# MayeulCassier/Matrix-Factorization-With-Comparison-Data

Hardware: AMD Instinct MI355X
Metric: triplet-updates/sec (higher is better)
Workload: dtype f32

## Files before the change

matrix-factorization-with-comparison-data_amd/csrc/resident.hip:

```cpp
#include <cstring>
#include <mutex>
#include <utility>
#include <vector>

#include "resident_kernel.h"

#define MFCD_DECL(d)                                                                                                  \
    extern "C" int mfcd_resident_launch_d##d(const mfcd_detail::ResidentArgs *, int, int, void *) __attribute__((weak)); \
    extern "C" int mfcd_resident_occupancy_d##d(int, int, int, int) __attribute__((weak));
MFCD_DECL(2) MFCD_DECL(4) MFCD_DECL(8) MFCD_DECL(16) MFCD_DECL(32) MFCD_DECL(64) MFCD_DECL(128) MFCD_DECL(256)
#undef MFCD_DECL

namespace mfcd_detail {

int g_resident_math = 1;
Tuning g_tune;

typedef int (*ResidentLauncher)(const ResidentArgs *, int, int, void *);
typedef int (*ResidentOccupancy)(int, int, int, int);

static ResidentLauncher launcher_for(int d)
{
    switch (d) {
        case 2: return mfcd_resident_launch_d2;
// ... 141 lines not shown
    for (int r = 0; r < 3; ++r) {
        bool first = true;
#pragma unroll
        for (int r2 = 0; r2 < r; ++r2) first = first && w[r2] != w[r];
        need[r] = first;
        unsigned own = 0u, rows = 0u;
#pragma unroll
        for (int r2 = r; r2 < 3; ++r2)
            if (w[r2] == w[r]) {
                own |= 1u << r2;
                rows |= lr[r2] << (10 * r2);
            }
        e[r] = make_uint4(((unsigned)k << 9) | (tl << 3) | own, rows, __float_as_uint(s.z), 0u);
        list[r] = (size_t)w[r] * (size_t)nch_cap + (size_t)c;
    }
    unsigned slot[3] = {0u, 0u, 0u}, slot_back[3] = {0u, 0u, 0u};
#pragma unroll
    for (int r = 0; r < 3; ++r) {
        if (need[r]) slot[r] = atomicAdd(ev_cnt + list[r], 1u);
        if (need[r] && copy_back) slot_back[r] = atomicAdd(ev_cnt + list[r] - 1, 1u);
    }
#pragma unroll
    for (int r = 0; r < 3; ++r) {
        if (need[r] && slot[r] < (unsigned)kEventCap - 1u) ev_ent[list[r] * kEventCap + slot[r]] = e[r];
        if (need[r] && copy_back && slot_back[r] < (unsigned)kEventCap - 1u)
            ev_ent[(list[r] - 1) * kEventCap + slot_back[r]] = e[r];
    }
}

int launch_train_prologue(const StageCopy &sc, const SampleTranslation *tr, hipStream_t st)
{
    static const SampleTranslation none{nullptr, 0, 1, 0, 0, 0, 0, 0, 0, nullptr, nullptr, nullptr};
    const SampleTranslation &t = tr ? *tr : none;
    const int units = (int)((sc.bytes + 15) / 16);
    const int64_t items = t.xs ? (t.N > units ? t.N : units) : units;
    constexpr int kPT = 64;
    const dim3 grid((unsigned)((items + kPT - 1) / kPT));
    if (units <= kInlineStageUnits) {
        InlineStage inl;
        std::memcpy(inl.v, sc.host, (size_t)units * 16);
        hipLaunchKernelGGL(train_prologue_kernel<true>, grid, dim3(kPT), 0, st, inl, (const uint4 *)nullptr,
                           (uint4 *)sc.dev, units, t.samples, t.N, t.B, t.n, t.m, t.rows_per_wave, t.tshift, t.look,
                           t.nch_cap, t.xs, t.ev_cnt, (uint4 *)t.ev_ent);
    } else {
        static const InlineStage no_inline{};
        hipLaunchKernelGGL(train_prologue_kernel<false>, grid, dim3(kPT), 0, st, no_inline, (const uint4 *)sc.devview,
                           (uint4 *)sc.dev, units, t.samples, t.N, t.B, t.n, t.m, t.rows_per_wave, t.tshift, t.look,
                           t.nch_cap, t.xs, t.ev_cnt, (uint4 *)t.ev_ent);
    }
    MFCD_HIP_TRY(hipGetLastError());
    return 0;
}

int launch_resident_steps(const ResidentPlan &pl, const void *cold_dev, const mfcd_sample *xs, int64_t N, int B, int n,
                          int m, int d, const StepScalars *sc_dev, const AdamStatic &ac, unsigned long long *mailbox,
                          unsigned tag_base, void *loss_terms, unsigned long long *dbg, int K, hipStream_t st)
{
    ResidentArgs a;
    a.dbg = dbg;
    a.cold = (const ResidentCold *)cold_dev;
    a.samples = xs; a.sc = sc_dev; a.mailbox = mailbox; a.loss_terms = loss_terms;
    a.N = N; a.B = B; a.n = n; a.m = m; a.K = K; a.NW = pl.NW; a.ac = ac;
    a.lookahead = pl.lookahead;
    a.tag_base = tag_base;
    a.fast_math = pl.fast_math;
    a.bf16 = pl.bf16;
    ResidentLauncher fn = launcher_for(d);
    if (!fn) return MFCD_EINVAL;
    return fn(&a, pl.Q, pl.blocks, (void *)st);
}

}
```

matrix-factorization-with-comparison-data_amd/csrc/resident_kernel.h:

```cpp
#pragma once
#include "common.h"
#include "train_common.h"

namespace mfcd_detail {

typedef unsigned long long u64;

#define MFCD_LAMBDA_INLINE __attribute__((always_inline))

#ifdef MFCD_RES_STATS
#define RS_NOW() ((u64)__builtin_amdgcn_s_memtime())
#define RS_ADD(slot, val) rs_acc[slot] += (u64)(val)
#else
#define RS_NOW() ((u64)0)
#define RS_ADD(slot, val) ((void)0)
#endif

typedef const __attribute__((address_space(4))) float *ScalarTablePtr;
__device__ __forceinline__ StepScalars load_step_scalars(const StepScalars *table, int k)
{
    const ScalarTablePtr f = (ScalarTablePtr)(table + k);
    StepScalars s;
    s.neg_step_size = f[0];
    s.bc2_sqrt = f[1];
    s.inv_bc2_sqrt = f[2];
    s.pad = 0.0f;
    return s;
}


__device__ __forceinline__ u64 pack_granule(unsigned tag, float v)
{
    return ((u64)tag << 32) | (u64)__float_as_uint(v);
}

__device__ __forceinline__ u64 load_granule(const u64 *p)
{
    return __hip_atomic_load(p, __ATOMIC_RELAXED, __HIP_MEMORY_SCOPE_AGENT);
}

__device__ __forceinline__ void store_granule(u64 *p, unsigned tag, float v)
{
    __hip_atomic_store(p, pack_granule(tag, v), __ATOMIC_RELAXED, __HIP_MEMORY_SCOPE_AGENT);
}

struct RowMap {
    int n, m, c;
    __host__ __device__ int vrow_u(int u) const { return u < c ? 2 * u : 2 * c + (u - c); }
    __host__ __device__ int vrow_v(int i) const { return i < c ? 2 * i + 1 : 2 * c + (i - c); }
    __host__ __device__ int users_below(int x) const
    {
        if (x <= 2 * c) return (x + 1) >> 1;
        return n > c ? c + (x - 2 * c) : c;
    }
    __host__ __device__ int items_below(int x) const
    {
        if (x <= 2 * c) return x >> 1;
        return m > c ? c + (x - 2 * c) : c;
    }
    __host__ __device__ bool is_item(int vr) const { return vr < 2 * c ? (vr & 1) != 0 : m > n; }
    __host__ __device__ int table_row(int vr) const { return vr < 2 * c ? vr >> 1 : c + (vr - 2 * c); }
};
__host__ __device__ inline RowMap make_row_map(int n, int m)
{
    RowMap r;
    r.n = n; r.m = m; r.c = n < m ? n : m;
    return r;
}

constexpr int kEventCap = 64;
constexpr unsigned kEventNone = 0xFFFFFFF8u;
constexpr int kEventMaxLocalRows = 1024;

struct ResidentArgs {
    const ResidentCold *cold;
    const mfcd_sample *samples;
    const StepScalars *sc;
    u64 *mailbox;
    void *loss_terms;
    u64 *dbg;
    unsigned tag_base;
    int64_t N;
    int B, n, m, K, NW;
    int lookahead;
    int fast_math;
    int bf16;
    AdamStatic ac;
};

__device__ __forceinline__ mfcd_sample load_record(const mfcd_sample *__restrict__ samples, int64_t pos0, int Bk,
                                                   int base, int lane)
{
    mfcd_sample s;
    s.u = s.i = s.j = -0x40000000;
    s.z = 0.0f;
    if (base + lane < Bk) s = samples[pos0 + base + lane];
    return s;
}

struct Masks {
    u64 mu, mi, mj;
};

template <int D, int Q, int LOOK, bool FAST, bool BF16 = false>
__global__ __launch_bounds__(256) __attribute__((amdgpu_waves_per_eu(Q >= 16 ? 2 : 1)))
void resident_train_kernel(ResidentArgs a)
{
    constexpr int S = D >= 64 ? D / 64 : 1;
    constexpr int RPR = D < 64 ? 64 / D : 1;
    constexpr int EW = 64 * Q;
    static_assert(EW % D == 0, "a wave's slice must hold whole rows");
    static_assert(EW / D <= kEventMaxLocalRows, "local row indices are 10-bit fields of an event entry");
    constexpr bool GRL = Q >= 16;
    extern __shared__ __attribute__((aligned(16))) float lds_dyn[];
    const int lane = threadIdx.x & 63;
    const int gw = blockIdx.x * (blockDim.x >> 6) + (threadIdx.x >> 6);
    if (gw >= a.NW) return;

    const int64_t T = (int64_t)(a.n + a.m) * D;
    const int64_t ebase = (int64_t)gw * EW;
    const int Rlo = (int)(ebase / D);
    const int64_t eend = (ebase + EW < T) ? ebase + EW : T;
    const int Rhi = (int)(eend / D);
    const int lcol = lane & (D - 1);
    auto elem_is_item = [&](int64_t e) MFCD_LAMBDA_INLINE { return make_row_map(a.n, a.m).is_item((int)(e / D)); };
    auto elem_offset = [&](int64_t e) MFCD_LAMBDA_INLINE { return (int64_t)make_row_map(a.n, a.m).table_row((int)(e / D)) * D + (e % D); };

#ifdef MFCD_RES_STATS
    u64 rs_acc[8] = {0, 0, 0, 0, 0, 0, 0, 0};
    const u64 rs_t0 = RS_NOW();
    [[maybe_unused]] const u64 rs_abs_t0 = __builtin_amdgcn_s_memrealtime();
    [[maybe_unused]] u64 rs_abs_l0 = 0, rs_abs_l1 = 0;
    [[maybe_unused]] u64 rs_hit[8] = {0, 0, 0, 0, 0, 0, 0, 0};
    [[maybe_unused]] u64 rs_mark = 0;
#endif
    float p[Q], m1[Q], m2[Q], gr[GRL ? 1 : Q];
    float *const lgr = lds_dyn + (threadIdx.x >> 6) * (GRL ? EW : 0);
    auto post = [](float x) MFCD_LAMBDA_INLINE {
        if constexpr (BF16) return (float)(mfcd_bf16)x;
        else return x;
    };
    {
        const ResidentCold c = *a.cold;
#pragma unroll
        for (int q = 0; q < Q; ++q) {
            const int64_t e = ebase + q * 64 + lane;
            p[q] = m1[q] = m2[q] = 0.0f;
            if constexpr (GRL) lgr[q * 64 + lane] = 0.0f;
            if (e < T) {
                const int64_t o = elem_offset(e);
                if (!elem_is_item(e)) { p[q] = BF16 ? (float)((const mfcd_bf16 *)c.U)[o] : c.U[o]; m1[q] = c.mU[o]; m2[q] = c.vU[o]; }
                else { p[q] = BF16 ? (float)((const mfcd_bf16 *)c.V)[o] : c.V[o]; m1[q] = c.mV[o]; m2[q] = c.vV[o]; }
            }
        }
    }

    auto batch_size = [&](int step) MFCD_LAMBDA_INLINE {
        const int64_t pos0 = (int64_t)step * a.B;
        return (int)((a.N - pos0) < a.B ? (a.N - pos0) : a.B);
    };
    auto scan = [&](const mfcd_sample &s, int Bk, int base) MFCD_LAMBDA_INLINE {
        const bool valid = base + lane < Bk;
        const int ru = s.u, ri = s.i, rj = s.j;
        Masks M;
        M.mu = __ballot(valid && ru >= Rlo && ru < Rhi);
        M.mi = __ballot(valid && ri >= Rlo && ri < Rhi);
        M.mj = __ballot(valid && rj >= Rlo && rj < Rhi);
        return M;
    };
    auto reg_of = [&](int lr) MFCD_LAMBDA_INLINE { return D >= 64 ? lr * S : lr / RPR; };

    auto give_up = [&](int step, int64_t pos, int what) MFCD_LAMBDA_INLINE {
        int *const status = a.cold->status;
        if (lane == 0) {
            if (__hip_atomic_exchange(status, 1, __ATOMIC_RELAXED, __HIP_MEMORY_SCOPE_AGENT) == 0 && a.dbg) {
                a.dbg[0] = (u64)gw; a.dbg[1] = (u64)step; a.dbg[2] = (u64)pos; a.dbg[3] = (u64)what;
            }
        }
    };
    auto poll_failed = [&](unsigned &spins, unsigned &limit) MFCD_LAMBDA_INLINE -> bool {
        if (spins == 0) limit = (unsigned)a.cold->spin_limit;
        ++spins;
        if (spins > limit || (spins & 255u) == 0) {
            if (spins > limit ||
                __hip_atomic_load(a.cold->status, __ATOMIC_RELAXED, __HIP_MEMORY_SCOPE_AGENT) != 0)
                return true;
        }
        return false;
    };

    auto store_row = [&](int lr, int64_t slot, unsigned tag) MFCD_LAMBDA_INLINE {
        u64 *dst = a.mailbox + slot * D;
        const int q0 = reg_of(lr);
#pragma unroll
        for (int q = 0; q < Q; ++q) {
            if (q >= q0 && q < q0 + S) {
                if constexpr (D >= 64) {
                    store_granule(dst + (q - q0) * 64 + lane, tag, p[q]);
                } else {
                    if (lane / D == lr % RPR) store_granule(dst + lcol, tag, p[q]);
                }
            }
        }
    };

    auto process_hit = [&](bool own0, bool own1, bool own2, int lr0, int lr1, int lr2, float zz, int64_t pos,
                           unsigned tag, float inv_batch, int step) MFCD_LAMBDA_INLINE -> bool {
        const bool own[3] = {own0, own1, own2};
        const int lrs[3] = {lr0, lr1, lr2};
        const u64 *slot = a.mailbox + pos * 3 * D;

        float row[3][S];
#pragma unroll
        for (int r = 0; r < 3; ++r) {
#pragma unroll
            for (int s2 = 0; s2 < S; ++s2) row[r][s2] = 0.0f;
            if (!own[r]) continue;
            const int q0 = reg_of(lrs[r]);
            if constexpr (D >= 64) {
#pragma unroll
                for (int q = 0; q < Q; ++q)
                    if (q >= q0 && q < q0 + S) row[r][(q * 64 % D) / 64] = p[q];
            } else {
                float sel = 0.0f;
#pragma unroll
                for (int q = 0; q < Q; ++q) sel = (q == q0) ? p[q] : sel;
                const float v = __shfl(sel, (lrs[r] % RPR) * D + lcol, MFCD_WAVE);
                row[r][0] = lane < D ? v : 0.0f;
            }
        }
        unsigned spins = 0, limit = 0;
        [[maybe_unused]] u64 rs_w0 = 0;
        RS_ADD(4, 1ull);
#ifdef MFCD_RES_STAMPS
        { const u64 t = RS_NOW(); rs_hit[0] += t - rs_mark; rs_mark = t; }
#endif
#if defined(MFCD_RES_STAGGER) && MFCD_RES_STAGGER > 0
        {
            u64 ga[3][S], gb[3][S];
            auto issue = [&](u64 (&g)[3][S]) MFCD_LAMBDA_INLINE {
#pragma unroll
                for (int r = 0; r < 3; ++r) {
                    if (own[r]) continue;
#pragma unroll
                    for (int s2 = 0; s2 < S; ++s2) {
                        const int c = lane + 64 * s2;
                        if (c < D) g[r][s2] = load_granule(slot + (int64_t)r * D + c);
                    }
                }
            };
            auto check = [&](const u64 (&g)[3][S]) MFCD_LAMBDA_INLINE -> bool {
                bool ok = true;
#pragma unroll
                for (int r = 0; r < 3; ++r) {
                    if (own[r]) continue;
#pragma unroll
                    for (int s2 = 0; s2 < S; ++s2) {
                        const int c = lane + 64 * s2;
                        if (c < D) {
                            ok = ok && ((unsigned)(g[r][s2] >> 32) == tag);
                            row[r][s2] = __uint_as_float((unsigned)g[r][s2]);
                        }
                    }
                }
                return __all(ok);
            };
            issue(ga);
            if (!check(ga)) {
#ifdef MFCD_RES_STATS
                rs_w0 = RS_NOW();
#endif
                issue(ga);
                __builtin_amdgcn_s_sleep(MFCD_RES_STAGGER);
                issue(gb);
                while (true) {
                    RS_ADD(5, 1);
                    if (poll_failed(spins, limit)) {
                        give_up(step, pos, (own0 ? 1 : 0) | (own1 ? 2 : 0) | (own2 ? 4 : 0));
                        return false;
                    }
                    if (check(ga)) break;
                    issue(ga);
                    if (check(gb)) break;
                    issue(gb);
                }
            }
        }
#else
        while (true) {
            bool ok = true;
#pragma unroll
            for (int r = 0; r < 3; ++r) {
                if (own[r]) continue;
#pragma unroll
                for (int s2 = 0; s2 < S; ++s2) {
                    const int c = lane + 64 * s2;
                    if (c < D) {
                        const u64 gq = load_granule(slot + (int64_t)r * D + c);
                        ok = ok && ((unsigned)(gq >> 32) == tag);
                        row[r][s2] = __uint_as_float((unsigned)gq);
                    }
                }
            }
            if (__all(ok)) break;
#ifdef MFCD_RES_STATS
            if (spins == 0) rs_w0 = RS_NOW();
            RS_ADD(5, 1);
#endif
            if (poll_failed(spins, limit)) {
                give_up(step, pos, (own0 ? 1 : 0) | (own1 ? 2 : 0) | (own2 ? 4 : 0));
                return false;
            }
        }
#endif
#ifdef MFCD_RES_STATS
        if (spins) RS_ADD(2, RS_NOW() - rs_w0);
        else RS_ADD(4, 1ull << 40);
#endif
#ifdef MFCD_RES_STAMPS
        { const u64 t = RS_NOW(); rs_hit[1] += t - rs_mark; if (!spins) { rs_hit[6] += t - rs_mark; rs_hit[7] += 1; } rs_mark = t; }
#endif

        float acc = 0.0f;
#pragma unroll
        for (int s2 = 0; s2 < S; ++s2) acc += row[0][s2] * (row[1][s2] - row[2][s2]);
        float pr, g;
        if constexpr (FAST) {
            const float x = wave_sum64(acc);
            const float e = __builtin_amdgcn_exp2f(x * -1.44269504088896340736f);
            const float dn = 1.0f + e;
            pr = div_newton(1.0f, dn, __builtin_amdgcn_rcpf(dn));
            pr = (e == __builtin_inff()) ? 0.0f : pr;
            const float den = fmaxf((1.0f - pr) * pr, 1e-12f);
            const float num = inv_batch * (pr - zz);
            g = div_newton(num, den, __builtin_amdgcn_rcpf(den)) * (1.0f - pr) * pr;
        } else {
            pr = sigmoid_f32(wave_sum64(acc));
            g = bce_sigmoid_backward_f32(pr, zz, inv_batch);
        }
        if (own[0] && lane == 0) {
            if constexpr (LOOK > 0) store_granule((u64 *)a.loss_terms + pos, tag, pr);
            else ((float *)a.loss_terms)[pos] = pr;
        }

        float du[S], dv[S];
#pragma unroll
        for (int s2 = 0; s2 < S; ++s2) {
            du[s2] = g * (row[1][s2] - row[2][s2]);
            dv[s2] = g * row[0][s2];
        }
        if constexpr (D < 64) {
            du[0] = __shfl(du[0], lcol, MFCD_WAVE);
            dv[0] = __shfl(dv[0], lcol, MFCD_WAVE);
        }
        if constexpr (GRL) {
#pragma unroll
            for (int r = 0; r < 3; ++r) {
                if (!own[r]) continue;
                const int q0 = reg_of(lrs[r]);
                if constexpr (D >= 64) {
#pragma unroll
                    for (int s2 = 0; s2 < S; ++s2)
                        lgr[(q0 + s2) * 64 + lane] += r == 0 ? du[s2] : (r == 1 ? dv[s2] : -dv[s2]);
                } else {
                    if (lane / D == lrs[r] % RPR) lgr[q0 * 64 + lane] += r == 0 ? du[0] : (r == 1 ? dv[0] : -dv[0]);
                }
            }
// ... 29 lines not shown
                    adam_update_t<FAST>(p[q], m1[q], m2[q], 0.0f, a.ac, sc);
                    p[q] = post(p[q]);
                }
            }
        } else {
            adam_update_q<FAST, Q, false>(p, m1, m2, gr, a.ac, sc);
            if constexpr (BF16) {
#pragma unroll
                for (int q = 0; q < Q; ++q) p[q] = post(p[q]);
            }
        }
    };

    auto generic_loop = [&]() MFCD_LAMBDA_INLINE -> bool {
        auto publish = [&](int step) MFCD_LAMBDA_INLINE {
            const int64_t pos0 = (int64_t)step * a.B;
            const int Bk = batch_size(step);
            for (int base = 0; base < Bk; base += MFCD_WAVE) {
                const mfcd_sample s = load_record(a.samples, pos0, Bk, base, lane);
                const Masks M = scan(s, Bk, base);
                u64 mask = M.mu | M.mi | M.mj;
                while (mask) {
                    const int tl = __ffsll((long long)mask) - 1;
                    mask &= mask - 1;
                    const int64_t slot0 = (pos0 + base + tl) * 3;
                    if ((M.mu >> tl) & 1ull) store_row(__shfl(s.u, tl, MFCD_WAVE) - Rlo, slot0 + 0, a.tag_base + (unsigned)step + 1u);
                    if ((M.mi >> tl) & 1ull) store_row(__shfl(s.i, tl, MFCD_WAVE) - Rlo, slot0 + 1, a.tag_base + (unsigned)step + 1u);
                    if ((M.mj >> tl) & 1ull) store_row(__shfl(s.j, tl, MFCD_WAVE) - Rlo, slot0 + 2, a.tag_base + (unsigned)step + 1u);
                }
            }
        };
        publish(0);
        for (int k = 0; k < a.K; ++k) {
            const int64_t pos0 = (int64_t)k * a.B;
            const int Bk = batch_size(k);
            const float inv_batch = 1.0f / (float)Bk;
            const StepScalars sc = load_step_scalars(a.sc, k);
            if constexpr (!GRL) {
#pragma unroll
                for (int q = 0; q < Q; ++q) gr[q] = 0.0f;
            }
            bool any_hit = false;
            for (int base = 0; base < Bk; base += MFCD_WAVE) {
                const mfcd_sample s = load_record(a.samples, pos0, Bk, base, lane);
                const Masks M = scan(s, Bk, base);
                u64 mask = M.mu | M.mi | M.mj;
                any_hit = any_hit || mask != 0ull;
                while (mask) {
                    const int tl = __ffsll((long long)mask) - 1;
                    mask &= mask - 1;
                    const int hu = __shfl(s.u, tl, MFCD_WAVE) - Rlo, hi = __shfl(s.i, tl, MFCD_WAVE) - Rlo,
                              hj = __shfl(s.j, tl, MFCD_WAVE) - Rlo;
                    const float hz = __shfl(s.z, tl, MFCD_WAVE);
                    const bool ok = process_hit((bool)((M.mu >> tl) & 1ull), (bool)((M.mi >> tl) & 1ull),
                                                (bool)((M.mj >> tl) & 1ull), hu, hi, hj, hz, pos0 + base + tl,
                                                a.tag_base + (unsigned)k + 1u, inv_batch, k);
                    if (__builtin_amdgcn_readfirstlane((int)!ok)) return false;
                }
            }
            step_update(any_hit, sc);
            if (k + 1 < a.K) publish(k + 1);
        }
        return true;
    };

    bool alive = true;

    if constexpr (LOOK > 0) {
        const int W = __builtin_amdgcn_readfirstlane(a.lookahead);
        const int N32 = (int)a.N;
        const int gws = __builtin_amdgcn_readfirstlane(gw);
        const int tshift = (int)a.cold->tshift;
        const int NCH = ((a.K - 1) >> tshift) + 1;

        bool fits = true;
        {
            const unsigned *cnt = a.cold->ev_cnt + (size_t)gws * (size_t)a.cold->nch_cap;
            for (int c = lane; c < NCH; c += MFCD_WAVE) fits = fits && cnt[c] < (unsigned)kEventCap;
            fits = __all(fits);
        }
        if (!__builtin_amdgcn_readfirstlane((int)fits)) {
            alive = generic_loop();
        } else {
            unsigned ekey = kEventNone, erow = 0u;
            int estep = 0x7FFFFF;
            float ez = 0.0f;
            int chunk_end = 0;

            auto load_chunk = [&](int c) MFCD_LAMBDA_INLINE {
                const ResidentCold *cz = a.cold;
                const size_t li = (size_t)gws * (size_t)cz->nch_cap + (size_t)c;
                const uint4 e = cz->ev_ent[li * kEventCap + lane];
                const unsigned n_raw = cz->ev_cnt[li];
                const unsigned n = (unsigned)__builtin_amdgcn_readfirstlane((int)n_raw);
                const unsigned key = (unsigned)lane < n ? e.x : kEventNone;
                unsigned rank = 0u;
                for (unsigned l = 0; l < n; ++l) {
                    const unsigned kl = (unsigned)__builtin_amdgcn_readlane((int)key, (int)l);
                    rank += kl < key ? 1u : 0u;
                }
                const int dest = (int)((unsigned)lane < n ? rank : (unsigned)lane) << 2;
                ekey = (unsigned)__builtin_amdgcn_ds_permute(dest, (int)key);
                erow = (unsigned)__builtin_amdgcn_ds_permute(dest, (int)e.y);
                ez = __builtin_bit_cast(float, __builtin_amdgcn_ds_permute(dest, (int)e.z));
                estep = (int)(ekey >> 9);
                const int ce = (c + 1) << tshift;
                chunk_end = ce < a.K ? ce : a.K;
            };
            auto step_at = [&](int i) MFCD_LAMBDA_INLINE -> int { return __builtin_amdgcn_readlane(estep, i); };
            auto lanes_in = [](int lo, int hi) MFCD_LAMBDA_INLINE -> u64 { return ((1ull << hi) - 1ull) & ~((1ull << lo) - 1ull); };
            auto rowmask = [&](int lr) MFCD_LAMBDA_INLINE -> u64 {
                const bool t = ((ekey & 1u) && (int)(erow & 1023u) == lr) ||
                               ((ekey & 2u) && (int)((erow >> 10) & 1023u) == lr) ||
                               ((ekey & 4u) && (int)((erow >> 20) & 1023u) == lr);
                return __ballot(t);
            };

            auto publish_entry = [&](int idx, int jbase, int conf_lo, int conf_hi, int touch_lo, int touch_hi,
                                     bool need_touch) MFCD_LAMBDA_INLINE {
                const unsigned key_l = (unsigned)__builtin_amdgcn_readlane((int)ekey, idx);
                const unsigned row_l = (unsigned)__builtin_amdgcn_readlane((int)erow, idx);
                const int ke = (int)(key_l >> 9);
                const int tl = (int)((key_l >> 3) & 63u);
#pragma unroll 1
                for (int r = 0; r < 3; ++r) {
                    if (!((key_l >> r) & 1u)) continue;
                    const int lr = (int)((row_l >> (10 * r)) & 1023u);
                    if (conf_lo < conf_hi || need_touch) {
                        const u64 rm = rowmask(lr);
                        if (rm & lanes_in(conf_lo, conf_hi)) continue;
                        if (need_touch && !(rm & lanes_in(touch_lo, touch_hi))) continue;
                    }
                    const int q0 = reg_of(lr);
                    float pp[S], mm1[S], mm2[S];
#pragma unroll
                    for (int s2 = 0; s2 < S; ++s2) pp[s2] = mm1[s2] = mm2[s2] = 0.0f;
#pragma unroll
                    for (int q = 0; q < Q; ++q) {
                        if (q >= q0 && q < q0 + S) {
                            const int s2 = D >= 64 ? (q * 64 % D) / 64 : 0;
                            pp[s2] = p[q];
                            mm1[s2] = m1[q];
                            mm2[s2] = m2[q];
                        }
                    }
                    StepScalars scb = load_step_scalars(a.sc, jbase + 1);
#pragma unroll 1
                    for (int st = jbase + 1; st < ke; ++st) {
                        const StepScalars scn = load_step_scalars(a.sc, st + 1);
#pragma unroll
                        for (int s2 = 0; s2 < S; ++s2) {
                            adam_update_t<FAST>(pp[s2], mm1[s2], mm2[s2], 0.0f, a.ac, scb);
                            pp[s2] = post(pp[s2]);
                        }
                        scb = scn;
                    }
                    u64 *dst = a.mailbox + (((int64_t)ke * a.B + tl) * 3 + r) * D;
                    const unsigned tag = a.tag_base + (unsigned)ke + 1u;
                    if constexpr (D >= 64) {
#pragma unroll
                        for (int s2 = 0; s2 < S; ++s2) store_granule(dst + s2 * 64 + lane, tag, pp[s2]);
                    } else {
                        if (lane / D == lr % RPR) store_granule(dst + lcol, tag, pp[0]);
                    }
                    RS_ADD(7, 1);
                }
            };
            auto publish_fresh = [&](int jbase, int lo, int hi, int touch_lo, int touch_hi) MFCD_LAMBDA_INLINE {
                if (lo >= hi) return;
                [[maybe_unused]] const u64 rs_p0 = RS_NOW();
                int g0 = lo, gstep = step_at(lo);
                for (int idx = lo; idx < hi; ++idx) {
                    const int st = step_at(idx);
                    if (st != gstep) { g0 = idx; gstep = st; }
                    publish_entry(idx, jbase, lo, g0, touch_lo, touch_hi, jbase >= 0);
                }
                RS_ADD(3, RS_NOW() - rs_p0);
            };
            load_chunk(0);
            int hc = 0, pc = __builtin_popcountll(__ballot(estep < W));
            publish_fresh(-1, 0, pc, 0, 0);
            int nh = step_at(0), np = step_at(pc);
            auto next_event = [&]() MFCD_LAMBDA_INLINE -> int {
                const int cp = np - W;
                const int e = nh < cp ? nh : cp;
                return e < chunk_end ? e : chunk_end;
            };
            int next_evt = next_event();

            ScalarTablePtr scp = (ScalarTablePtr)a.sc;
            auto load_scalars_at = [&](ScalarTablePtr f) MFCD_LAMBDA_INLINE {
                StepScalars x;
                x.neg_step_size = f[0];
                x.bc2_sqrt = f[1];
                x.inv_bc2_sqrt = f[2];
                x.pad = 0.0f;
                return x;
            };
            StepScalars sc_cur = load_scalars_at(scp);
            int chunk = 0;
#ifdef MFCD_RES_STATS
            const u64 rs_l0 = RS_NOW();
            rs_acc[6] = rs_l0 - rs_t0;
            rs_abs_l0 = __builtin_amdgcn_s_memrealtime();
#endif
            int k = 0;
            while (true) {
                const int kq = next_evt < a.K ? next_evt : a.K;
                while (k < kq) {
                    scp += 4;
                    const StepScalars sc_next = load_scalars_at(scp);
                    if constexpr (GRL) {
                        step_update(false, sc_cur);
                    } else {
#pragma unroll
                        for (int q = 0; q < Q; ++q) {
                            adam_update_t<FAST>(p[q], m1[q], m2[q], 0.0f, a.ac, sc_cur);
                            p[q] = post(p[q]);
                        }
                    }
                    sc_cur = sc_next;
                    ++k;
                }
                if (k >= a.K) break;
                scp += 4;
                const StepScalars sc_next = load_scalars_at(scp);
                if constexpr (!GRL) {
#pragma unroll
                    for (int q = 0; q < Q; ++q) gr[q] = 0.0f;
                }
                bool hit = false;
                int h0 = 0;
                {
                    __builtin_amdgcn_s_setprio(3);
                    [[maybe_unused]] const u64 rs_e0 = RS_NOW();
#ifdef MFCD_RES_STAMPS
                    rs_mark = rs_e0;
#endif
                    RS_ADD(7, 1ull << 32);
                    if (k == chunk_end) {
                        load_chunk(++chunk);
                        hc = 0;
                        nh = step_at(0);
                        pc = __builtin_popcountll(__ballot(estep < k + W));
                        np = step_at(pc);
                    }
                    if (np == k + W) {
                        [[maybe_unused]] const u64 rs_p0 = RS_NOW();
                        const int g0 = pc;
                        do {
                            publish_entry(pc, k - 1, hc, g0, 0, 0, false);
                            ++pc;
                            np = step_at(pc);
                        } while (np == k + W);
                        RS_ADD(3, RS_NOW() - rs_p0);
                    }
                    h0 = hc;
                    if (nh == k) {
                        hit = true;
                        const int bk = (N32 - k * a.B) < a.B ? (N32 - k * a.B) : a.B;
                        const float inv_batch = 1.0f / (float)bk;
                        const unsigned tag = a.tag_base + (unsigned)k + 1u;
                        do {
                            const unsigned key_l = (unsigned)__builtin_amdgcn_readlane((int)ekey, hc);
                            const unsigned row_l = (unsigned)__builtin_amdgcn_readlane((int)erow, hc);
                            const float z_l = __builtin_bit_cast(float, __builtin_amdgcn_readlane(__builtin_bit_cast(int, ez), hc));
                            const bool ok = process_hit((bool)(key_l & 1u), (bool)(key_l & 2u), (bool)(key_l & 4u),
                                                        (int)(row_l & 1023u), (int)((row_l >> 10) & 1023u),
                                                        (int)((row_l >> 20) & 1023u), z_l,
                                                        (int64_t)k * a.B + (int)((key_l >> 3) & 63u), tag, inv_batch, k);
                            if (__builtin_amdgcn_readfirstlane((int)!ok)) { alive = false; break; }
                            ++hc;
                            nh = step_at(hc);
                        } while (nh == k);
                        if (!alive) break;
                    }
                    next_evt = next_event();
                    if (!hit) __builtin_amdgcn_s_setprio(0);
                    RS_ADD(1, RS_NOW() - rs_e0);
                }
                step_update(hit, sc_cur);
#ifdef MFCD_RES_STAMPS
                if (hit) { const u64 t = RS_NOW(); rs_hit[3] += t - rs_mark; rs_mark = t; }
#endif
                if (__builtin_expect(hit, 0)) {
                    publish_fresh(k, hc, pc, h0, hc);
                    __builtin_amdgcn_s_setprio(0);
#ifdef MFCD_RES_STAMPS
                    { const u64 t = RS_NOW(); rs_hit[4] += t - rs_mark; rs_hit[5] += 1; }
#endif
                }
                sc_cur = sc_next;
                ++k;
            }
            __builtin_amdgcn_s_setprio(0);
#ifdef MFCD_RES_STATS
            rs_abs_l1 = __builtin_amdgcn_s_memrealtime();
            rs_acc[0] = RS_NOW() - rs_l0;
            rs_acc[6] |= (u64)__builtin_amdgcn_s_getreg((31 << 11) | 4) << 32;
            rs_acc[5] |= (u64)__builtin_amdgcn_s_getreg((31 << 11) | 20) << 32;
            if (lane == 0 && a.dbg)
                for (int x = 0; x < 8; ++x) a.dbg[8 + (int64_t)gw * 8 + x] = rs_acc[x];
#endif
        }

        {
            float *const loss_out = a.cold->loss_out;
            if (loss_out != nullptr) {
                for (int k = gws; k < a.K && alive; k += a.NW) {
                    const int64_t off = (int64_t)k * a.B;
                    const int b = (int)((a.N - off) < a.B ? (a.N - off) : a.B);
                    const unsigned tag = a.tag_base + (unsigned)k + 1u;
                    const float zz = lane < b ? a.samples[off + lane].z : 0.0f;
                    unsigned spins = 0, limit = 0;
                    float pr = 0.0f;
                    while (true) {
                        bool ok = true;
                        if (lane < b) {
                            const u64 gq = load_granule((const u64 *)a.loss_terms + off + lane);
                            ok = (unsigned)(gq >> 32) == tag;
                            pr = __uint_as_float((unsigned)gq);
                        }
                        if (__all(ok)) break;
                        __builtin_amdgcn_s_sleep(8);
                        if (poll_failed(spins, limit)) {
                            give_up(k, off, 8);
                            alive = false;
                            break;
                        }
                    }
                    if (!alive) break;
                    float acc = lane < b ? bce_term_f32(pr, zz) : 0.0f;
                    acc = wave_sum64(acc);
                    if (lane == 0) loss_out[k] = acc / (float)b;
                }
            }
        }
        {
            unsigned *const cnt = a.cold->ev_cnt + (size_t)gws * (size_t)a.cold->nch_cap;
            for (int c = lane; c < NCH; c += MFCD_WAVE) cnt[c] = 0u;
        }
    } else {
        alive = generic_loop();
    }

    const ResidentCold c = *a.cold;
#pragma unroll
    for (int q = 0; q < Q; ++q) {
        const int64_t e = ebase + q * 64 + lane;
        if (e < T) {
            const int64_t o = elem_offset(e);
            if (!elem_is_item(e)) {
                if constexpr (BF16) ((mfcd_bf16 *)c.U)[o] = (mfcd_bf16)p[q];
                else c.U[o] = p[q];
                c.mU[o] = m1[q]; c.vU[o] = m2[q];
            } else {
                if constexpr (BF16) ((mfcd_bf16 *)c.V)[o] = (mfcd_bf16)p[q];
                else c.V[o] = p[q];
                c.mV[o] = m1[q]; c.vV[o] = m2[q];
            }
        }
    }
#ifdef MFCD_RES_STAMPS
    if (lane == 0 && a.dbg) {
        u64 *const o = a.dbg + 8 + (int64_t)gw * 8;
        o[1] = rs_abs_t0; o[2] = rs_abs_l0; o[3] = rs_abs_l1; o[7] = __builtin_amdgcn_s_memrealtime();
        for (int x = 0; x < 8; ++x) o[4096 * 8 + x] = rs_hit[x];
    }
#endif
}

}
```

matrix-factorization-with-comparison-data_amd/csrc/train.hip:

```cpp
#include <cstring>
#include <memory>
#include <mutex>
#include <unordered_map>
#include <vector>

#include "common.h"
#include "train_common.h"

namespace {

int g_train_path = 0;

int device_cus()
{
    static int cached = 0;
    if (!cached) {
        int dev = 0, cus = 0;
        if (hipGetDevice(&dev) == hipSuccess &&
            hipDeviceGetAttribute(&cus, hipDeviceAttributeMultiprocessorCount, dev) == hipSuccess && cus > 0)
            cached = cus;
        else {
            (void)hipGetLastError();
            cached = 256;
        }
// ... 311 lines not shown
    if (g_train_path == 0 && local_ok) {
        c.form = 3;
        return c;
    }
    bool resident_ok = false;
    if (resident_planned && g_train_path != 1 && N > 0 && nsteps <= 0x7fffffff &&
        nsteps + 1 < ((int64_t)1 << kTagStepBits)) {
        c.rp = mfcd_detail::plan_resident(N, B, n, m, d, device_cus(), !f32, ev_tshift);
        resident_ok = c.rp.ok;
    }
    if (g_train_path == 2) {
        c.form = resident_ok ? 2 : MFCD_EINVAL;
        return c;
    }
    c.form = (resident_ok && nsteps >= kShortCallSteps) ? 2 : 1;
    return c;
}

struct TrainCall {
    AdamTables t;
    int bf16, B, n, m, d;
    AdamHyper h;
    void *workspace;
    size_t workspace_bytes;
};

int run_persistent(WsState &S, const TrainCall &c, const FormChoice &fc, const mfcd_sample *samples, int64_t N,
                   int64_t step0, float *loss_per_step, hipStream_t st, float *timing_us, bool stage_only)
{
    using mfcd_detail::ResidentCold;
    const TrainLayout &L = S.L;
    const int B = c.B, n = c.n, m = c.m, d = c.d;
    const int64_t nsteps = (N + B - 1) / B;
    char *base = (char *)c.workspace;
    const bool resident = fc.form == 2;
    const bool means_inside = resident && fc.rp.lookahead > 0;
    const WsState::Staged call{true, samples, c.t.U, N, step0, loss_per_step, c.h.lr, c.h.beta1, c.h.beta2, 0};
    bool staged_hit = false;
    const int set = S.claim_set(call, means_inside && !timing_us, stage_only, &staged_hit);
    const PrologueRegions &R = L.set[set];
    ResidentCold *cold_dev = (ResidentCold *)(base + R.stage_off);
    const StepScalars *sc_dev = (const StepScalars *)(cold_dev + 1);
    const mfcd_detail::SampleTranslation tr{samples, N, B, n, m, resident ? 64 * fc.rp.Q / d : 0, fc.rp.tshift,
                                            means_inside ? fc.rp.lookahead : 0, L.nch_cap,
                                            resident ? (mfcd_sample *)(base + R.xs_off) : nullptr,
                                            (unsigned *)(base + R.evcnt_off), base + R.event_off};
    const size_t need = kColdBytes + sizeof(StepScalars) * (size_t)(nsteps + 1);
    alignas(16) unsigned char inline_stage[4096];
    const bool stage_inline = need <= mfcd_detail::train_inline_stage_bytes() && need <= sizeof(inline_stage);
    StageSlot *slot = nullptr;
    if (!staged_hit && !stage_inline)
        if (int rc = stage_acquire(S, need, &slot)) return rc;
    char *const stage_host = slot ? (char *)slot->host : (char *)inline_stage;
    if (!staged_hit) {
        ResidentCold cold{};
        cold.U = (float *)c.t.U; cold.V = (float *)c.t.V;
        cold.mU = c.t.mU; cold.vU = c.t.vU; cold.mV = c.t.mV; cold.vV = c.t.vV;
        cold.status = (int *)base; cold.spin_limit = mfcd_detail::g_tune.spin_limit;
        cold.ev_cnt = tr.ev_cnt; cold.ev_ent = (uint4 *)tr.ev_ent;
        cold.nch_cap = L.nch_cap; cold.tshift = fc.rp.tshift;
        cold.loss_out = means_inside ? loss_per_step : nullptr;
        std::memcpy(stage_host, &cold, sizeof(cold));
        StepScalars *sc_host = (StepScalars *)(stage_host + sizeof(cold));
        for (int64_t k = 0; k <= nsteps; ++k) sc_host[k] = step_scalars(c.h, step0 + k + 1);
        if (means_inside)
            if (int rc = S.clear_lists(set, base, st)) return rc;
    }
    unsigned tag_base = 0;
    if (!stage_only) {
        if (resident) {
            if (int rc = S.next_tag_base(base, st, &tag_base)) return rc;
            if (int rc = S.clear_dirty(base, st)) return rc;
        }
        if (!means_inside) S.terms_dirty = true;
    }
    if (!staged_hit) {
        if (stage_only) S.lists_dirty[set] = true;
        if (int rc = mfcd_detail::launch_train_prologue({stage_host, slot ? slot->devview : nullptr, cold_dev, need},
                                                        &tr, st))
            return rc;
    }
    if (stage_only) {
        if (slot)
            if (int rc = slot->release(st)) return rc;
        S.staged = call;
        S.staged.set = set;
        return 0;
    }
    if (staged_hit) S.staged.valid = false;
    if (resident) {
        S.last_set = set;
        S.lists_dirty[set] = false;
    }

    hipEvent_t e0 = nullptr, e1 = nullptr;
    if (timing_us) {
        MFCD_HIP_TRY(hipEventCreate(&e0));
        MFCD_HIP_TRY(hipEventCreate(&e1));
        MFCD_HIP_TRY(hipEventRecord(e0, st));
    }
    const AdamStatic as = adam_static(c.h);
    void *terms = base + L.terms_off;
    int rc = 0;
    if (resident)
        rc = mfcd_detail::launch_resident_steps(fc.rp, cold_dev, tr.xs, N, B, n, m, d, sc_dev, as,
                                                (unsigned long long *)(base + L.mailbox_off), tag_base, terms,
                                                (unsigned long long *)(base + L.dbg_off), (int)nsteps, st);
    else
        rc = mfcd_detail::launch_local_steps((float *)c.t.U, (float *)c.t.V, c.t.mU, c.t.vU, c.t.mV, c.t.vV, samples, N, B,
                                             n, m, d, sc_dev, as, (float *)terms, (int)nsteps, st);
    if (rc) return rc;
    if (timing_us) MFCD_HIP_TRY(hipEventRecord(e1, st));
    if (loss_per_step && !means_inside)
        rc = mfcd_detail::launch_batch_means((const float *)terms, samples, N, B, loss_per_step, st);
    if (rc) return rc;
    if (slot)
        if (int rc = slot->release(st)) return rc;
    if (timing_us) {
        MFCD_HIP_TRY(hipEventSynchronize(e1));
        float ms = 0.0f;
        MFCD_HIP_TRY(hipEventElapsedTime(&ms, e0, e1));
        timing_us[0] = timing_us[1] = timing_us[2] = ms * 1e3f / (float)nsteps;
        (void)hipEventDestroy(e0);
        (void)hipEventDestroy(e1);
    }
    return 0;
}

template <typename TP>
int run_streaming(WsState &S, const TrainCall &c, const mfcd_sample *samples, int64_t N, int64_t step0,
                  float *loss_per_step, hipStream_t st, float *timing_us)
{
    const TrainLayout &L = S.L;
    const int B = c.B, n = c.n, m = c.m, d = c.d;
    const int64_t nsteps = (N + B - 1) / B;
    char *base = (char *)c.workspace;
    TP *U = (TP *)c.t.U, *V = (TP *)c.t.V;
    if (L.resident) S.mailbox_dirty = S.terms_dirty = true;
    TP *Ualt = (TP *)(base + L.ualt_off);
    TP *Valt = (TP *)(base + L.valt_off);
    float *terms = (float *)(base + L.terms_off);

    const void *ptrs[] = {U, V, c.t.mU, c.t.vU, c.t.mV, c.t.vV, Ualt, Valt};
    const mfcd_detail::Plan pl = mfcd_detail::make_plan(ptrs, 8, n, m, d);
    std::vector<hipEvent_t> ev;
    if (timing_us) {
        ev.resize(2 * (size_t)nsteps);
        for (auto &e : ev) MFCD_HIP_TRY(hipEventCreate(&e));
    }
    for (int64_t k = 0; k < nsteps; ++k) {
        const int64_t off = k * B;
        const int Bk = (int)((N - off) < B ? (N - off) : B);
        const AdamConst ac = adam_const(c.h, step0 + k + 1);
        const bool even = (k & 1) == 0;
        if (timing_us) MFCD_HIP_TRY(hipEventRecord(ev[2 * k], st));
        mfcd_detail::launch_streaming_step<0, TP>(pl, st, even ? U : Ualt, even ? V : Valt, even ? Ualt : U,
                                                  even ? Valt : V, c.t.mU, c.t.vU, c.t.mV, c.t.vV, samples + off,
                                                  nullptr, Bk, 1.0f / (float)Bk, n, m, d, ac, terms + off);
// ... 329 lines not shown
```

matrix-factorization-with-comparison-data_amd/csrc/train_common.h:

```cpp
#pragma once
#include "common.h"

struct AdamStatic {
    float w1;
    float b2;
    float w2;
    float eps;
    float wd;
};

struct StepScalars {
    float neg_step_size;
    float bc2_sqrt;
    float inv_bc2_sqrt;
    float pad;
};

struct AdamConst {
    AdamStatic st;
    StepScalars sc;
};

struct AdamHyper { double lr, beta1, beta2, eps, wd; };
struct AdamTables {
// ... 225 lines not shown
int set_uvt_min_stages(int v);

struct ResidentSlices {
    int count;
    struct { int Q, waves; } at[5];
};
ResidentSlices resident_slices(int n, int m, int d, int num_cus);

ResidentPlan plan_resident(int64_t N, int B, int n, int m, int d, int num_cus, bool bf16 = false, int ev_tshift = -1);
int resident_lookahead(int64_t N, int B, int n, int m);

struct ResidentEvents {
    int tshift;
    int waves;
    int rows_per_wave;
};
ResidentEvents resident_events(int B, int n, int m, int d, int num_cus);
constexpr int kResidentEventCap = 64;
constexpr int kResidentEventLook = 16;
inline int64_t resident_event_chunks(int64_t K, int tshift) { return (K >> tshift) + 2; }

size_t train_inline_stage_bytes();

struct ResidentCold {
    float *U, *V, *mU, *vU, *mV, *vV;
    int *status;
    unsigned long long spin_limit;
    unsigned *ev_cnt;
    uint4 *ev_ent;
    long long nch_cap;
    long long tshift;
    float *loss_out;
    unsigned long long pad[3];
};
static_assert(sizeof(ResidentCold) == 128, "eight 16-byte units of the stage table (resident.hip: kInlineStageUnits)");

struct StageCopy {
    const void *host;
    const void *devview;
    void *dev;
    size_t bytes;
};
struct SampleTranslation {
    const mfcd_sample *samples;
    int64_t N;
    int B, n, m, rows_per_wave, tshift, look;
    int64_t nch_cap;
    mfcd_sample *xs;
    unsigned *ev_cnt;
    void *ev_ent;
};
int launch_train_prologue(const StageCopy &sc, const SampleTranslation *tr, hipStream_t st);

int launch_resident_steps(const ResidentPlan &pl, const void *cold_dev, const mfcd_sample *xs, int64_t N, int B, int n,
                          int m, int d, const StepScalars *sc_dev, const AdamStatic &ac, unsigned long long *mailbox,
                          unsigned tag_base, void *loss_terms, unsigned long long *dbg, int K, hipStream_t st);
constexpr int kResidentMaxWaves = 4096;

}
```

Measured before the change: 92.22 million.

## Pass cold args by kernarg, prefetch mailbox granules for upcoming hits

Moves the ResidentCold pointer table out of a device buffer and into the kernel arguments, read through the kernarg segment pointer, so it no longer costs a global load on each access. It also prefetches the first event chunk before the fits check, and issues mailbox granule loads for up to two upcoming hits at the start of a step, before the chunk reload and other work. This hides the mailbox load latency behind that work. The price is more registers for the two granule buffers, and the old stagger path is removed.

```diff
diff --git a/matrix-factorization-with-comparison-data_amd/csrc/resident.hip b/matrix-factorization-with-comparison-data_amd/csrc/resident.hip
--- a/matrix-factorization-with-comparison-data_amd/csrc/resident.hip
+++ b/matrix-factorization-with-comparison-data_amd/csrc/resident.hip
@@ -217,13 +217,13 @@
     return 0;
 }
 
-int launch_resident_steps(const ResidentPlan &pl, const void *cold_dev, const mfcd_sample *xs, int64_t N, int B, int n,
+int launch_resident_steps(const ResidentPlan &pl, const ResidentCold &cold, const mfcd_sample *xs, int64_t N, int B, int n,
                           int m, int d, const StepScalars *sc_dev, const AdamStatic &ac, unsigned long long *mailbox,
                           unsigned tag_base, void *loss_terms, unsigned long long *dbg, int K, hipStream_t st)
 {
     ResidentArgs a;
     a.dbg = dbg;
-    a.cold = (const ResidentCold *)cold_dev;
+    a.cv = cold;
     a.samples = xs; a.sc = sc_dev; a.mailbox = mailbox; a.loss_terms = loss_terms;
     a.N = N; a.B = B; a.n = n; a.m = m; a.K = K; a.NW = pl.NW; a.ac = ac;
     a.lookahead = pl.lookahead;
diff --git a/matrix-factorization-with-comparison-data_amd/csrc/resident_kernel.h b/matrix-factorization-with-comparison-data_amd/csrc/resident_kernel.h
--- a/matrix-factorization-with-comparison-data_amd/csrc/resident_kernel.h
+++ b/matrix-factorization-with-comparison-data_amd/csrc/resident_kernel.h
@@ -73,7 +73,7 @@
 constexpr int kEventMaxLocalRows = 1024;
 
 struct ResidentArgs {
-    const ResidentCold *cold;
+    ResidentCold cv;
     const mfcd_sample *samples;
     const StepScalars *sc;
     u64 *mailbox;
@@ -140,8 +140,21 @@
         if constexpr (BF16) return (float)(mfcd_bf16)x;
         else return x;
     };
+    auto cold_args = [&]() MFCD_LAMBDA_INLINE -> ResidentCold {
+        typedef const __attribute__((address_space(4))) char *KernargPtr;
+        KernargPtr ka = (KernargPtr)__builtin_amdgcn_kernarg_segment_ptr();
+        asm volatile("" : "+s"(ka));
+        ka += offsetof(ResidentArgs, cv);
+        ResidentCold c{};
+#define MFCD_COLD_FIELD(f) c.f = *(const __attribute__((address_space(4))) decltype(c.f) *)(ka + offsetof(ResidentCold, f))
+        MFCD_COLD_FIELD(U); MFCD_COLD_FIELD(V); MFCD_COLD_FIELD(mU); MFCD_COLD_FIELD(vU); MFCD_COLD_FIELD(mV);
+        MFCD_COLD_FIELD(vV); MFCD_COLD_FIELD(status); MFCD_COLD_FIELD(spin_limit); MFCD_COLD_FIELD(ev_cnt);
+        MFCD_COLD_FIELD(ev_ent); MFCD_COLD_FIELD(nch_cap); MFCD_COLD_FIELD(tshift); MFCD_COLD_FIELD(loss_out);
+#undef MFCD_COLD_FIELD
+        return c;
+    };
+    const ResidentCold cs = cold_args();
     {
-        const ResidentCold c = *a.cold;
 #pragma unroll
         for (int q = 0; q < Q; ++q) {
             const int64_t e = ebase + q * 64 + lane;
@@ -149,8 +162,8 @@
             if constexpr (GRL) lgr[q * 64 + lane] = 0.0f;
             if (e < T) {
                 const int64_t o = elem_offset(e);
-                if (!elem_is_item(e)) { p[q] = BF16 ? (float)((const mfcd_bf16 *)c.U)[o] : c.U[o]; m1[q] = c.mU[o]; m2[q] = c.vU[o]; }
-                else { p[q] = BF16 ? (float)((const mfcd_bf16 *)c.V)[o] : c.V[o]; m1[q] = c.mV[o]; m2[q] = c.vV[o]; }
+                if (!elem_is_item(e)) { p[q] = BF16 ? (float)((const mfcd_bf16 *)cs.U)[o] : cs.U[o]; m1[q] = cs.mU[o]; m2[q] = cs.vU[o]; }
+                else { p[q] = BF16 ? (float)((const mfcd_bf16 *)cs.V)[o] : cs.V[o]; m1[q] = cs.mV[o]; m2[q] = cs.vV[o]; }
             }
         }
     }
@@ -171,7 +184,7 @@
     auto reg_of = [&](int lr) MFCD_LAMBDA_INLINE { return D >= 64 ? lr * S : lr / RPR; };
 
     auto give_up = [&](int step, int64_t pos, int what) MFCD_LAMBDA_INLINE {
-        int *const status = a.cold->status;
+        int *const status = cold_args().status;
         if (lane == 0) {
             if (__hip_atomic_exchange(status, 1, __ATOMIC_RELAXED, __HIP_MEMORY_SCOPE_AGENT) == 0 && a.dbg) {
                 a.dbg[0] = (u64)gw; a.dbg[1] = (u64)step; a.dbg[2] = (u64)pos; a.dbg[3] = (u64)what;
@@ -179,11 +192,11 @@
         }
     };
     auto poll_failed = [&](unsigned &spins, unsigned &limit) MFCD_LAMBDA_INLINE -> bool {
-        if (spins == 0) limit = (unsigned)a.cold->spin_limit;
+        if (spins == 0) limit = (unsigned)cold_args().spin_limit;
         ++spins;
         if (spins > limit || (spins & 255u) == 0) {
             if (spins > limit ||
-                __hip_atomic_load(a.cold->status, __ATOMIC_RELAXED, __HIP_MEMORY_SCOPE_AGENT) != 0)
+                __hip_atomic_load(cold_args().status, __ATOMIC_RELAXED, __HIP_MEMORY_SCOPE_AGENT) != 0)
                 return true;
         }
         return false;
@@ -204,11 +217,23 @@
         }
     };
 
+    auto issue_hit = [&](bool own0, bool own1, bool own2, int64_t pos, u64 (&g)[3][S]) MFCD_LAMBDA_INLINE {
+        const bool own[3] = {own0, own1, own2};
+        const u64 *slot = a.mailbox + pos * 3 * D;
+#pragma unroll
+        for (int r = 0; r < 3; ++r) {
+            if (own[r]) continue;
+#pragma unroll
+            for (int s2 = 0; s2 < S; ++s2) {
+                const int c = lane + 64 * s2;
+                if (c < D) g[r][s2] = load_granule(slot + (int64_t)r * D + c);
+            }
+        }
+    };
     auto process_hit = [&](bool own0, bool own1, bool own2, int lr0, int lr1, int lr2, float zz, int64_t pos,
-                           unsigned tag, float inv_batch, int step) MFCD_LAMBDA_INLINE -> bool {
+                           unsigned tag, float inv_batch, int step, u64 (&gl)[3][S], bool have) MFCD_LAMBDA_INLINE -> bool {
         const bool own[3] = {own0, own1, own2};
         const int lrs[3] = {lr0, lr1, lr2};
-        const u64 *slot = a.mailbox + pos * 3 * D;
 
         float row[3][S];
 #pragma unroll
@@ -233,61 +258,11 @@
         [[maybe_unused]] u64 rs_w0 = 0;
         RS_ADD(4, 1ull);
 #ifdef MFCD_RES_STAMPS
-        { const u64 t = RS_NOW(); rs_hit[0] += t - rs_mark; rs_mark = t; }
-#endif
-#if defined(MFCD_RES_STAGGER) && MFCD_RES_STAGGER > 0
-        {
-            u64 ga[3][S], gb[3][S];
-            auto issue = [&](u64 (&g)[3][S]) MFCD_LAMBDA_INLINE {
-#pragma unroll
-                for (int r = 0; r < 3; ++r) {
-                    if (own[r]) continue;
-#pragma unroll
-                    for (int s2 = 0; s2 < S; ++s2) {
-                        const int c = lane + 64 * s2;
-                        if (c < D) g[r][s2] = load_granule(slot + (int64_t)r * D + c);
-                    }
-                }
-            };
-            auto check = [&](const u64 (&g)[3][S]) MFCD_LAMBDA_INLINE -> bool {
-                bool ok = true;
-#pragma unroll
-                for (int r = 0; r < 3; ++r) {
-                    if (own[r]) continue;
-#pragma unroll
-                    for (int s2 = 0; s2 < S; ++s2) {
-                        const int c = lane + 64 * s2;
-                        if (c < D) {
-                            ok = ok && ((unsigned)(g[r][s2] >> 32) == tag);
-                            row[r][s2] = __uint_as_float((unsigned)g[r][s2]);
-                        }
-                    }
-                }
-                return __all(ok);
-            };
-            issue(ga);
-            if (!check(ga)) {
-#ifdef MFCD_RES_STATS
-                rs_w0 = RS_NOW();
-#endif
-                issue(ga);
-                __builtin_amdgcn_s_sleep(MFCD_RES_STAGGER);
-                issue(gb);
-                while (true) {
-                    RS_ADD(5, 1);
-                    if (poll_failed(spins, limit)) {
-                        give_up(step, pos, (own0 ? 1 : 0) | (own1 ? 2 : 0) | (own2 ? 4 : 0));
-                        return false;
-                    }
-                    if (check(ga)) break;
-                    issue(ga);
-                    if (check(gb)) break;
-                    issue(gb);
-                }
-            }
-        }
-#else
+        if (!have) { const u64 t = RS_NOW(); rs_hit[0] += t - rs_mark; rs_mark = t; }
+#endif
         while (true) {
+            if (!have) issue_hit(own0, own1, own2, pos, gl);
+            have = false;
             bool ok = true;
 #pragma unroll
             for (int r = 0; r < 3; ++r) {
@@ -296,7 +271,7 @@
                 for (int s2 = 0; s2 < S; ++s2) {
                     const int c = lane + 64 * s2;
                     if (c < D) {
-                        const u64 gq = load_granule(slot + (int64_t)r * D + c);
+                        const u64 gq = gl[r][s2];
                         ok = ok && ((unsigned)(gq >> 32) == tag);
                         row[r][s2] = __uint_as_float((unsigned)gq);
                     }
@@ -312,7 +287,6 @@
                 return false;
             }
         }
-#endif
 #ifdef MFCD_RES_STATS
         if (spins) RS_ADD(2, RS_NOW() - rs_w0);
         else RS_ADD(4, 1ull << 40);
@@ -448,9 +422,10 @@
                     const int hu = __shfl(s.u, tl, MFCD_WAVE) - Rlo, hi = __shfl(s.i, tl, MFCD_WAVE) - Rlo,
                               hj = __shfl(s.j, tl, MFCD_WAVE) - Rlo;
                     const float hz = __shfl(s.z, tl, MFCD_WAVE);
+                    u64 gran[3][S];
                     const bool ok = process_hit((bool)((M.mu >> tl) & 1ull), (bool)((M.mi >> tl) & 1ull),
                                                 (bool)((M.mj >> tl) & 1ull), hu, hi, hj, hz, pos0 + base + tl,
-                                                a.tag_base + (unsigned)k + 1u, inv_batch, k);
+                                                a.tag_base + (unsigned)k + 1u, inv_batch, k, gran, false);
                     if (__builtin_amdgcn_readfirstlane((int)!ok)) return false;
                 }
             }
@@ -466,13 +441,16 @@
         const int W = __builtin_amdgcn_readfirstlane(a.lookahead);
         const int N32 = (int)a.N;
         const int gws = __builtin_amdgcn_readfirstlane(gw);
-        const int tshift = (int)a.cold->tshift;
+        const int tshift = (int)cs.tshift;
         const int NCH = ((a.K - 1) >> tshift) + 1;
 
+        const size_t list0 = (size_t)gws * (size_t)cs.nch_cap;
+        const uint4 ent0 = cs.ev_ent[list0 * kEventCap + lane];
+        const unsigned cnt0 = cs.ev_cnt[list0];
         bool fits = true;
         {
-            const unsigned *cnt = a.cold->ev_cnt + (size_t)gws * (size_t)a.cold->nch_cap;
-            for (int c = lane; c < NCH; c += MFCD_WAVE) fits = fits && cnt[c] < (unsigned)kEventCap;
+            const unsigned *cnt = cs.ev_cnt + list0;
+            for (int ch = lane; ch < NCH; ch += MFCD_WAVE) fits = fits && cnt[ch] < (unsigned)kEventCap;
             fits = __all(fits);
         }
         if (!__builtin_amdgcn_readfirstlane((int)fits)) {
@@ -483,11 +461,7 @@
             float ez = 0.0f;
             int chunk_end = 0;
 
-            auto load_chunk = [&](int c) MFCD_LAMBDA_INLINE {
-                const ResidentCold *cz = a.cold;
-                const size_t li = (size_t)gws * (size_t)cz->nch_cap + (size_t)c;
-                const uint4 e = cz->ev_ent[li * kEventCap + lane];
-                const unsigned n_raw = cz->ev_cnt[li];
+            auto sort_chunk = [&](int c, const uint4 &e, unsigned n_raw) MFCD_LAMBDA_INLINE {
                 const unsigned n = (unsigned)__builtin_amdgcn_readfirstlane((int)n_raw);
                 const unsigned key = (unsigned)lane < n ? e.x : kEventNone;
                 unsigned rank = 0u;
@@ -502,6 +476,13 @@
                 estep = (int)(ekey >> 9);
                 const int ce = (c + 1) << tshift;
                 chunk_end = ce < a.K ? ce : a.K;
+            };
+            auto load_chunk = [&](int c) MFCD_LAMBDA_INLINE {
+                const ResidentCold cz = cold_args();
+                const size_t li = (size_t)gws * (size_t)cz.nch_cap + (size_t)c;
+                const uint4 e = cz.ev_ent[li * kEventCap + lane];
+                const unsigned n_raw = cz.ev_cnt[li];
+                sort_chunk(c, e, n_raw);
             };
             auto step_at = [&](int i) MFCD_LAMBDA_INLINE -> int { return __builtin_amdgcn_readlane(estep, i); };
             auto lanes_in = [](int lo, int hi) MFCD_LAMBDA_INLINE -> u64 { return ((1ull << hi) - 1ull) & ~((1ull << lo) - 1ull); };
@@ -573,7 +554,7 @@
                 }
                 RS_ADD(3, RS_NOW() - rs_p0);
             };
-            load_chunk(0);
+            sort_chunk(0, ent0, cnt0);
             int hc = 0, pc = __builtin_popcountll(__ballot(estep < W));
             publish_fresh(-1, 0, pc, 0, 0);
             int nh = step_at(0), np = step_at(pc);
@@ -634,6 +615,21 @@
                     rs_mark = rs_e0;
 #endif
                     RS_ADD(7, 1ull << 32);
+                    u64 ga[3][S], gb[3][S];
+                    unsigned ka_key = kEventNone, kb_key = kEventNone;
+                    if (nh == k) {
+                        ka_key = (unsigned)__builtin_amdgcn_readlane((int)ekey, hc);
+                        issue_hit((bool)(ka_key & 1u), (bool)(ka_key & 2u), (bool)(ka_key & 4u),
+                                  (int64_t)k * a.B + (int)((ka_key >> 3) & 63u), ga);
+                        if (step_at(hc + 1) == k) {
+                            kb_key = (unsigned)__builtin_amdgcn_readlane((int)ekey, hc + 1);
+                            issue_hit((bool)(kb_key & 1u), (bool)(kb_key & 2u), (bool)(kb_key & 4u),
+                                      (int64_t)k * a.B + (int)((kb_key >> 3) & 63u), gb);
+                        }
+#ifdef MFCD_RES_STAMPS
+                        { const u64 t = RS_NOW(); rs_hit[0] += t - rs_mark; rs_mark = t; }
+#endif
+                    }
                     if (k == chunk_end) {
                         load_chunk(++chunk);
                         hc = 0;
@@ -664,8 +660,17 @@
                             const bool ok = process_hit((bool)(key_l & 1u), (bool)(key_l & 2u), (bool)(key_l & 4u),
                                                         (int)(row_l & 1023u), (int)((row_l >> 10) & 1023u),
                                                         (int)((row_l >> 20) & 1023u), z_l,
-                                                        (int64_t)k * a.B + (int)((key_l >> 3) & 63u), tag, inv_batch, k);
+                                                        (int64_t)k * a.B + (int)((key_l >> 3) & 63u), tag, inv_batch, k,
+                                                        ga, ka_key == key_l);
                             if (__builtin_amdgcn_readfirstlane((int)!ok)) { alive = false; break; }
+                            ka_key = kb_key;
+                            if (kb_key != kEventNone) {
+#pragma unroll
+                                for (int r = 0; r < 3; ++r)
+#pragma unroll
+                                    for (int s2 = 0; s2 < S; ++s2) ga[r][s2] = gb[r][s2];
+                                kb_key = kEventNone;
+                            }
                             ++hc;
                             nh = step_at(hc);
                         } while (nh == k);
@@ -701,7 +706,7 @@
         }
 
         {
-            float *const loss_out = a.cold->loss_out;
+            float *const loss_out = cold_args().loss_out;
             if (loss_out != nullptr) {
                 for (int k = gws; k < a.K && alive; k += a.NW) {
                     const int64_t off = (int64_t)k * a.B;
@@ -733,14 +738,15 @@
             }
         }
         {
-            unsigned *const cnt = a.cold->ev_cnt + (size_t)gws * (size_t)a.cold->nch_cap;
-            for (int c = lane; c < NCH; c += MFCD_WAVE) cnt[c] = 0u;
+            const ResidentCold cz = cold_args();
+            unsigned *const cnt = cz.ev_cnt + (size_t)gws * (size_t)cz.nch_cap;
+            for (int ch = lane; ch < NCH; ch += MFCD_WAVE) cnt[ch] = 0u;
         }
     } else {
         alive = generic_loop();
     }
 
-    const ResidentCold c = *a.cold;
+    const ResidentCold c = cold_args();
 #pragma unroll
     for (int q = 0; q < Q; ++q) {
         const int64_t e = ebase + q * 64 + lane;
diff --git a/matrix-factorization-with-comparison-data_amd/csrc/train.hip b/matrix-factorization-with-comparison-data_amd/csrc/train.hip
--- a/matrix-factorization-with-comparison-data_amd/csrc/train.hip
+++ b/matrix-factorization-with-comparison-data_amd/csrc/train.hip
@@ -387,14 +387,14 @@
     if (!staged_hit && !stage_inline)
         if (int rc = stage_acquire(S, need, &slot)) return rc;
     char *const stage_host = slot ? (char *)slot->host : (char *)inline_stage;
+    ResidentCold cold{};
+    cold.U = (float *)c.t.U; cold.V = (float *)c.t.V;
+    cold.mU = c.t.mU; cold.vU = c.t.vU; cold.mV = c.t.mV; cold.vV = c.t.vV;
+    cold.status = (int *)base; cold.spin_limit = mfcd_detail::g_tune.spin_limit;
+    cold.ev_cnt = tr.ev_cnt; cold.ev_ent = (uint4 *)tr.ev_ent;
+    cold.nch_cap = L.nch_cap; cold.tshift = fc.rp.tshift;
+    cold.loss_out = means_inside ? loss_per_step : nullptr;
     if (!staged_hit) {
-        ResidentCold cold{};
-        cold.U = (float *)c.t.U; cold.V = (float *)c.t.V;
-        cold.mU = c.t.mU; cold.vU = c.t.vU; cold.mV = c.t.mV; cold.vV = c.t.vV;
-        cold.status = (int *)base; cold.spin_limit = mfcd_detail::g_tune.spin_limit;
-        cold.ev_cnt = tr.ev_cnt; cold.ev_ent = (uint4 *)tr.ev_ent;
-        cold.nch_cap = L.nch_cap; cold.tshift = fc.rp.tshift;
-        cold.loss_out = means_inside ? loss_per_step : nullptr;
         std::memcpy(stage_host, &cold, sizeof(cold));
         StepScalars *sc_host = (StepScalars *)(stage_host + sizeof(cold));
         for (int64_t k = 0; k <= nsteps; ++k) sc_host[k] = step_scalars(c.h, step0 + k + 1);
@@ -438,7 +438,7 @@
     void *terms = base + L.terms_off;
     int rc = 0;
     if (resident)
-        rc = mfcd_detail::launch_resident_steps(fc.rp, cold_dev, tr.xs, N, B, n, m, d, sc_dev, as,
+        rc = mfcd_detail::launch_resident_steps(fc.rp, cold, tr.xs, N, B, n, m, d, sc_dev, as,
                                                 (unsigned long long *)(base + L.mailbox_off), tag_base, terms,
                                                 (unsigned long long *)(base + L.dbg_off), (int)nsteps, st);
     else
diff --git a/matrix-factorization-with-comparison-data_amd/csrc/train_common.h b/matrix-factorization-with-comparison-data_amd/csrc/train_common.h
--- a/matrix-factorization-with-comparison-data_amd/csrc/train_common.h
+++ b/matrix-factorization-with-comparison-data_amd/csrc/train_common.h
@@ -301,7 +301,7 @@
 };
 int launch_train_prologue(const StageCopy &sc, const SampleTranslation *tr, hipStream_t st);
 
-int launch_resident_steps(const ResidentPlan &pl, const void *cold_dev, const mfcd_sample *xs, int64_t N, int B, int n,
+int launch_resident_steps(const ResidentPlan &pl, const ResidentCold &cold, const mfcd_sample *xs, int64_t N, int B, int n,
                           int m, int d, const StepScalars *sc_dev, const AdamStatic &ac, unsigned long long *mailbox,
                           unsigned tag_base, void *loss_terms, unsigned long long *dbg, int K, hipStream_t st);
 constexpr int kResidentMaxWaves = 4096;
```

After: 98.90 million, median of 6. 7.2% higher.
